# mazouziwissem/improving_yolov8_CBAM_SwinBlock

Hardware: AMD Instinct MI355X
Metric: images/sec fwd+bwd YOLOv8s-CBAM-Swin bs=32 640x640 (higher is better)
Workload: dtype bf16; 1 GPU; yolov8s.yaml (nc=1) forward + v8 loss + backward + clip + SGD-nesterov + EMA step, bs=32/GPU 640x640 (CBAM + 2x SwinBlock + SPPF5 + SPPF7); global_batch=32, imgsz=640, parallelism=dp1

## Files before the change

improving_yolov8_cbam_swinblock_amd/_lib.py:

```python
import ctypes
import os
import subprocess
import threading
from pathlib import Path

import torch

PKG_DIR = Path(__file__).resolve().parent
CSRC_DIR = PKG_DIR / "csrc"
LIB_PATH = Path(os.environ["YMI_LIB"]).resolve() if os.environ.get("YMI_LIB") else PKG_DIR / "libyolo_mi355.so"

YMI_F32, YMI_BF16 = 0, 1
ACT_NONE, ACT_SILU, ACT_GELU = 0, 1, 2

_c_i64 = ctypes.c_int64
_c_i32 = ctypes.c_int32
_c_f32 = ctypes.c_float
_vp = ctypes.c_void_p
_sz = ctypes.c_size_t


class YmiTensor(ctypes.Structure):
    _fields_ = [
        ("data", _vp),
# ... 51 lines not shown
    ),
    "ymi_first_conv_stat_blocks": (_c_i64, [_c_i64, _c_i64, _c_i64]),
    "ymi_first_conv_bn_act_fwd": (_c_i32, [_vp, _c_i64, _c_i64, _c_i64, _c_i64, _vp, _c_i64, _vp, _vp, _vp, _vp, _c_f32, _c_f32, _c_i32, _TP, _TP, _vp, _vp,
                                           _vp, _sz, _vp]),
    "ymi_first_conv_bwd_workspace": (_c_i64, [_c_i64, _c_i64, _c_i64, _c_i64]),
    "ymi_first_conv_bn_act_bwd": (_c_i32, [_TP, _vp, _c_i64, _c_i64, _vp, _vp, _vp, _vp, _c_i32, _TP, _vp, _vp, _vp, _vp, _sz, _vp, _vp]),
    "ymi_bn_act_bwd_pair": (_c_i32, [_TP, _TP, _vp, _vp, _vp, _vp, _c_i64, _vp, _vp, _c_i32, _TP, _vp, _vp, _vp, _sz, _vp]),
    "ymi_conv2d_bwd_data": (_c_i32, [_TP, _vp, _c_i64, _c_i64, _c_i64, _c_i64, _TP, _vp]),
    "ymi_conv2d_bwd_data_add": (_c_i32, [_TP, _vp, _c_i64, _c_i64, _c_i64, _c_i64, _TP, _TP, _TP, _vp]),
    "ymi_swin_mlp_fwd": (_c_i32, [_TP, _vp, _vp, _c_i64, _vp, _vp, _TP, _TP, _TP, _TP, _vp]),
    "ymi_swin_ln_mlp_supported": (_c_i32, [_c_i64, _c_i64, _c_i32]),
    "ymi_swin_ln_mlp_pack_elems": (_c_i64, [_c_i64, _c_i64]),
    "ymi_swin_ln_mlp_pre_elems": (_c_i64, [_c_i64, _c_i64]),
    "ymi_swin_ln_mlp_pack": (_c_i32, [_vp, _vp, _c_i64, _c_i64, _vp, _vp]),
    "ymi_swin_ln_mlp_fwd": (_c_i32, [_TP, _vp, _vp, _c_f32, _vp, _vp, _vp, _c_i64, _TP, _vp, _vp, _vp, _TP, _vp]),
    "ymi_swin_ln_mlp_bwd_data": (_c_i32, [_TP, _vp, _vp, _c_i64, _TP, _TP, _TP, _vp]),
    "ymi_swin_mlp_bwd_data": (_c_i32, [_TP, _vp, _TP, _TP, _vp, _TP, _TP, _TP, _vp]),
    "ymi_conv2d_bwd_weight": (_c_i32, [_TP, _TP, _c_i64, _c_i64, _c_i64, _c_i64, _c_i64, _vp, _vp, _vp, _sz, _vp]),
    "ymi_conv2d_bwd_weight_workspace": (_sz, [_c_i64, _c_i64, _c_i64, _c_i64, _c_i64]),
    "ymi_conv2d_bwd_weight_deferred": (_c_i32, [_TP, _TP, _c_i64, _c_i64, _c_i64, _c_i64, _c_i64, _vp, _vp, _vp, _sz, _vp, _vp]),
    "ymi_wgrad_hold": (_c_i32, [_c_i32]),
    "ymi_wgrad_reduce_batch": (_c_i32, [_vp, _c_i32, _vp, _vp]),
    "ymi_sppf_pool3_fwd": (_c_i32, [_TP, _c_i64, _TP, _TP, _TP, _vp]),
    "ymi_sppf_pool3_bwd_workspace": (_c_i64, [_c_i64, _c_i64, _c_i64, _c_i64, _c_i32]),
    "ymi_sppf_pool3_bwd": (_c_i32, [_TP, _TP, _TP, _c_i64, _TP, _TP, _TP, _TP, _TP, _vp, _c_i64, _vp]),
    "ymi_cbam_fwd": (_c_i32, [_TP, _vp, _vp, _c_i64, _vp, _c_i64, _TP, _vp, _vp, _vp, _vp, _vp, _vp, _vp]),
    "ymi_cbam_bwd": (_c_i32, [_TP, _TP, _vp, _vp, _c_i64, _vp, _c_i64, _vp, _vp, _vp, _vp, _vp, _vp, _TP, _vp, _vp, _vp, _vp, _sz, _vp]),
    "ymi_cbam_bwd_workspace": (_sz, [_c_i64, _c_i64, _c_i64, _c_i64, _c_i64]),
    "ymi_window_partition_index": (_c_i32, [_c_i64, _c_i64, _c_i64, _c_i64, _vp, _vp]),
    "ymi_window_partition": (_c_i32, [_TP, _c_i64, _TP, _vp]),
# ... 217 lines not shown
```

improving_yolov8_cbam_swinblock_amd/csrc/common.h:

```cpp
#pragma once
#include <hip/hip_runtime.h>
#include <stdint.h>
#include <stdio.h>

#include "../../include/ymi.h"

typedef __bf16 bf16_t;
typedef __attribute__((ext_vector_type(8))) __bf16 bf16x8;
typedef __attribute__((ext_vector_type(4))) __bf16 bf16x4;
typedef __attribute__((ext_vector_type(4))) float f32x4;
typedef __attribute__((ext_vector_type(2))) float f32x2;
typedef __attribute__((ext_vector_type(4))) uint32_t u32x4;
typedef __attribute__((ext_vector_type(2))) uint32_t u32x2;

typedef const __attribute__((address_space(1))) void* gptr_t;
typedef __attribute__((address_space(3))) void* lptr_t;

#define YMI_WAVE 64

void ymi_set_error(const char* fmt, ...);
#define YMI_CHECK_ARG(cond, ...)          \
    do {                                  \
        if (!(cond)) {                    \
            ymi_set_error(__VA_ARGS__);   \
// ... 325 lines not shown

template <int N> __device__ __forceinline__ void wait_vmcnt_barrier() {
    asm volatile("s_waitcnt vmcnt(%0)\n\ts_barrier" ::"n"(N) : "memory");
}

__device__ __forceinline__ float wave_sum(float v) {
#pragma unroll
    for (int o = 32; o > 0; o >>= 1) v += __shfl_xor(v, o, 64);
    return v;
}
__device__ __forceinline__ float wave_max(float v) {
#pragma unroll
    for (int o = 32; o > 0; o >>= 1) v = fmaxf(v, __shfl_xor(v, o, 64));
    return v;
}
```

improving_yolov8_cbam_swinblock_amd/csrc/swin.hip:

```cpp
#include <stdlib.h>

#include <type_traits>

#include "common.h"

struct SV {
    const void* p;
    int64_t ld;
};

__device__ __forceinline__ int64_t token_pixel(int64_t t64, int H, int W, int Hp, int Wp, int ws, bool* real) {
    const uint32_t t = (uint32_t)t64, L = (uint32_t)(ws * ws), uws = (uint32_t)ws;
    const uint32_t nww = (uint32_t)Wp / uws, nwh = (uint32_t)Hp / uws;
    const uint32_t win = t / L, tok = t - win * L;
    const uint32_t wrow = win / nww, ww = win - wrow * nww;
    const uint32_t b = wrow / nwh, wh = wrow - b * nwh;
    const uint32_t tr = tok / uws;
    const int h = (int)(wh * uws + tr), w = (int)(ww * uws + (tok - tr * uws));
    *real = (h < H) && (w < W);
    return ((int64_t)b * H + h) * W + w;
}

__global__ void window_index_kernel(int64_t T, int Hp, int Wp, int ws, int* __restrict__ out) {
    for (int64_t t = blockIdx.x * (int64_t)blockDim.x + threadIdx.x; t < T; t += (int64_t)gridDim.x * blockDim.x) {
        bool real;
        out[t] = (int)token_pixel(t, Hp, Wp, Hp, Wp, ws, &real);
    }
}

extern "C" int ymi_window_partition_index(int64_t n, int64_t hp, int64_t wp, int64_t ws, int32_t* index, void* stream) {
    YMI_CHECK_ARG(index && ws > 0 && hp % ws == 0 && wp % ws == 0 && n > 0, "window_partition_index: args");
    const int64_t T = n * hp * wp;
    YMI_CHECK_ARG(T < (1ll << 31), "window_partition_index: too many tokens");
    hipLaunchKernelGGL(window_index_kernel, dim3((unsigned)((T + 255) / 256 > 4096 ? 4096 : (T + 255) / 256)), dim3(256), 0, (hipStream_t)stream,
                       T, (int)hp, (int)wp, (int)ws, index);
    YMI_CHECK_LAUNCH("window_partition_index");
// ... 377 lines not shown

struct AttnLds {
    size_t stage;
    int nstage, nsq;
    size_t sq;
    bool tail;
    constexpr size_t region(int i) const { return (size_t)i * stage; }
    constexpr size_t square(int i) const { return (size_t)nstage * stage + (size_t)i * sq; }
    constexpr size_t floats() const { return square(nsq); }
    constexpr size_t bytes() const { return floats() + (tail ? 64 * sizeof(float) : 0); }
};
template <typename T> constexpr AttnLds attn_one_tile_lds(int hdp, bool bwd) {
    const int rows = 64 * attn_row_bytes<T>(hdp), cols = hdp * attn_row_bytes<T>(64);
    return AttnLds{(size_t)(rows > cols ? rows : cols), 2, bwd ? 3 : 1, (size_t)64 * attn_row_bytes<T>(64), bwd};
}
constexpr AttnLds attn_tr_lds(int hdp, bool bwd) {
    return AttnLds{(size_t)64 * attn_row_bytes<bf16_t>(hdp), bwd ? 4 : 3, bwd ? 2 : 1, (size_t)64 * attn_row_bytes<bf16_t>(64), false};
}
template <typename T> constexpr AttnLds attn_tiled_lds(int nsq) {
    constexpr int rows = 64 * attn_row_bytes<T>(ATT_HC), cols = ATT_HC * attn_row_bytes<T>(64);
    return AttnLds{(size_t)(rows > cols ? rows : cols), 2, nsq, (size_t)64 * attn_row_bytes<T>(64), true};
}
static_assert(attn_one_tile_lds<float>(attn_hdp(16 * ATT_MAXDT), true).bytes() <= ATT_LDS_MAX, "one-tile float32 backward image exceeds the LDS");
static_assert(attn_tr_lds(attn_hdp(16 * ATT_MAXDT), true).bytes() <= ATT_LDS_MAX, "tr backward image exceeds the LDS");
static_assert(attn_one_tile_lds<float>(192, true).bytes() == 156928 && attn_tr_lds(192, true).bytes() == 120832, "tests/attn_exact.py attn_lds restates these");
static_assert(attn_tiled_lds<float>(2).bytes() <= ATT_LDS_MAX, "tiled dK/dV image exceeds the LDS");

__device__ __forceinline__ void attn_softmax_row(f32x4 (&s)[4], int nkeys, float scale, float m_run, int l4, float& mx, float& sum) {
    mx = m_run;
#pragma unroll
    for (int t = 0; t < 4; ++t)
#pragma unroll
        for (int r = 0; r < 4; ++r) {
            const int j = 16 * t + 4 * l4 + r;
            s[t][r] = j < nkeys ? s[t][r] * scale : -__builtin_inff();
            mx = fmaxf(mx, s[t][r]);
        }
    mx = fmaxf(mx, __shfl_xor(mx, 16, 64));
    mx = fmaxf(mx, __shfl_xor(mx, 32, 64));
    sum = 0.f;
// ... 253 lines not shown
        }
    }
}

__global__ __launch_bounds__(256) void window_attn_fwd_tr_kernel(AttnArgs a) {
    typedef bf16_t T;
    extern __shared__ __attribute__((aligned(16))) char smem[];
    const int lane = threadIdx.x & 63, wv = threadIdx.x >> 6;
    const int l15 = lane & 15, l4 = lane >> 4;
    const int hdp = a.hdp, L = a.L;
    const int rstride = attn_row_bytes<T>(hdp), tstride = attn_row_bytes<T>(64);
    const AttnLds lds = attn_tr_lds(hdp, false);
    char* Qs = smem + lds.region(0);
    char* Ks = smem + lds.region(1);
    char* Vs = smem + lds.region(2);
    char* P = smem + lds.square(0);
    const int head = blockIdx.y;
    const int co = head * a.hd;
    const int64_t t0 = (int64_t)blockIdx.x * L;
    const T* qkv = reinterpret_cast<const T*>(a.qkv.p) + t0 * a.qkv.ld;
    T* out = reinterpret_cast<T*>(const_cast<void*>(a.out.p)) + t0 * a.out.ld;
    const int ndt = (a.hd + 15) / 16;
    const bool vec4 = (a.hd & 3) == 0 && (a.out.ld & 3) == 0 && (((uintptr_t)a.out.p) & 7) == 0;
    {
        const bf16_t* srcs[3] = {qkv + co, qkv + a.C + co, qkv + 2 * a.C + co};
        const int64_t lds_[3] = {a.qkv.ld, a.qkv.ld, a.qkv.ld};
        char* dsts[3] = {Qs, Ks, Vs};
        attn_stage_rows<3>(srcs, lds_, dsts, L, a.hd, hdp);
    }
    __syncthreads();
    f32x4 s[4];
#pragma unroll
    for (int t = 0; t < 4; ++t) {
        s[t] = f32x4{0.f, 0.f, 0.f, 0.f};
        AT<T>::mma(Ks, rstride, t * 16, Qs, rstride, wv * 16, hdp, lane, s[t]);
    }
    float mx, sum;
    attn_softmax_row(s, L, a.scale, -__builtin_inff(), l4, mx, sum);
    const float inv = 1.f / sum;
    const int m = 16 * wv + l15;
    if (l4 == 0 && m < L && a.lse) a.lse[(t0 + m) * a.heads + head] = mx + __logf(sum);
#pragma unroll
    for (int t = 0; t < 4; ++t) {
        float p[4];
#pragma unroll
        for (int r = 0; r < 4; ++r) p[r] = s[t][r] * inv;
        Pack<T, 4>::store(reinterpret_cast<T*>(P + (size_t)m * tstride) + 16 * t + 4 * l4, p);
    }
    __syncthreads();
#pragma unroll
    for (int dt = 0; dt < ATT_MAXDT; ++dt)
        if (dt < ndt) {
            f32x4 o = f32x4{0.f, 0.f, 0.f, 0.f};
#pragma unroll
            for (int k0 = 0; k0 < 64; k0 += 32) {
                const bf16x8 af = *reinterpret_cast<const bf16x8*>(P + (size_t)(16 * wv + l15) * tstride + (k0 + 8 * l4) * 2);
// ... 4 lines not shown
        }
}

__global__ __launch_bounds__(256) void window_attn_bwd_tr_kernel(AttnArgs a) {
    typedef bf16_t T;
    extern __shared__ __attribute__((aligned(16))) char smem[];
    const int lane = threadIdx.x & 63, wv = threadIdx.x >> 6;
    const int l15 = lane & 15, l4 = lane >> 4;
    const int hdp = a.hdp, L = a.L;
    const int rstride = attn_row_bytes<T>(hdp), tstride = attn_row_bytes<T>(64);
    const AttnLds lds = attn_tr_lds(hdp, true);
    char* Qs = smem + lds.region(0);
    char* Ks = smem + lds.region(1);
    char* Vs = smem + lds.region(2);
    char* Os = smem + lds.region(3);
    char* Ps = smem + lds.square(0);
    char* Ds = smem + lds.square(1);
    const int head = blockIdx.y;
    const int co = head * a.hd;
    const int64_t t0 = (int64_t)blockIdx.x * L;
    const T* qkv = reinterpret_cast<const T*>(a.qkv.p) + t0 * a.qkv.ld;
    const T* dO = reinterpret_cast<const T*>(a.dout.p) + t0 * a.dout.ld;
    T* dqkv = reinterpret_cast<T*>(const_cast<void*>(a.dqkv.p)) + t0 * a.dqkv.ld;
    const int ndt = (a.hd + 15) / 16;
    const bool vec4 = (a.hd & 3) == 0 && (a.C & 3) == 0 && (a.dqkv.ld & 3) == 0 && (((uintptr_t)a.dqkv.p) & 7) == 0;

    const int mrow = 16 * wv + l15;
    const float lse = mrow < L ? a.lse[(t0 + mrow) * a.heads + head] : 0.f;
    {
        const bf16_t* srcs[4] = {qkv + co, qkv + a.C + co, qkv + 2 * a.C + co, dO + co};
        const int64_t lds_[4] = {a.qkv.ld, a.qkv.ld, a.qkv.ld, a.dout.ld};
        char* dsts[4] = {Qs, Ks, Vs, Os};
// ... 7 lines not shown
        dp[t] = f32x4{0.f, 0.f, 0.f, 0.f};
        AT<T>::mma(Ks, rstride, t * 16, Qs, rstride, wv * 16, hdp, lane, s[t]);
        AT<T>::mma(Vs, rstride, t * 16, Os, rstride, wv * 16, hdp, lane, dp[t]);
    }
    float pr[4][4], delta = 0.f;
#pragma unroll
    for (int t = 0; t < 4; ++t)
#pragma unroll
        for (int r = 0; r < 4; ++r) {
            const bool ok = (16 * t + 4 * l4 + r < L) && (mrow < L);
            pr[t][r] = ok ? __expf(s[t][r] * a.scale - lse) : 0.f;
            delta += pr[t][r] * dp[t][r];
        }
    delta += __shfl_xor(delta, 16, 64);
    delta += __shfl_xor(delta, 32, 64);
#pragma unroll
    for (int t = 0; t < 4; ++t) {
        float ds[4];
#pragma unroll
        for (int r = 0; r < 4; ++r) ds[r] = pr[t][r] * (dp[t][r] - delta) * a.scale;
        Pack<T, 4>::store(reinterpret_cast<T*>(Ps + (size_t)mrow * tstride) + 16 * t + 4 * l4, pr[t]);
        Pack<T, 4>::store(reinterpret_cast<T*>(Ds + (size_t)mrow * tstride) + 16 * t + 4 * l4, ds);
    }
    __syncthreads();
#pragma unroll
    for (int dt = 0; dt < ATT_MAXDT; ++dt)
        if (dt < ndt) {
            f32x4 dv = f32x4{0.f, 0.f, 0.f, 0.f}, dk = dv, dq = dv;
#pragma unroll
            for (int k0 = 0; k0 < 64; k0 += 32) {
// ... 324 lines not shown
```

improving_yolov8_cbam_swinblock_amd/csrc/swin_mlp.hip:

```cpp
#include <type_traits>

#include "common.h"

typedef __attribute__((ext_vector_type(16))) float f32x16;

template <int I, int N, class F> __device__ __forceinline__ void static_for(F&& f) {
    if constexpr (I < N) {
        f(std::integral_constant<int, I>{});
        static_for<I + 1, N>(f);
    }
}

constexpr int MLP_PAD = 256;
constexpr int MLP_HC = 32;
constexpr int MLP_LDS_MAX = 160 * 1024;
template <int C> struct MlpCfg {
    static_assert(C == 128 || C == 256 || C == 384, "SwinBlock widths of the model files");
    static constexpr int NW = C > 256 ? 4 : 8;
    static constexpr int WPS = NW / 4;
    static constexpr bool HALVES = NW == 8;
    static constexpr int NT = NW * 64;
    static constexpr int BM = NW * 32;
    static constexpr int KS = C / 16;
    static constexpr int CT = C / 32;
// ... 37 lines not shown
    const float* gamma;
    const float* beta;
    float eps;
    const bf16_t* w1p;
    const bf16_t* w2q;
    const float* b1;
    const float* b2;
    bf16_t* u;
    int64_t ldu;
    float* mean;
    float* rstd;
    bf16_t* pre;
    bf16_t* out;
    int64_t ldo;
    int T, hidden;
};

__device__ __forceinline__ uint32_t pack_bf16x2(float a, float b) {
    typedef __attribute__((ext_vector_type(2))) __bf16 bf16x2;
    const bf16x2 v = {(bf16_t)a, (bf16_t)b};
    return __builtin_bit_cast(uint32_t, v);
}
__device__ __forceinline__ float bf16_lo(uint32_t v) { return __builtin_bit_cast(float, v << 16); }
__device__ __forceinline__ float bf16_hi(uint32_t v) { return __builtin_bit_cast(float, v & 0xffff0000u); }

__device__ __forceinline__ float gelu_fast(float x, float* half_erfc = nullptr, float* e_out = nullptr) {
    const float ax = fabsf(x);
    const float t = __builtin_amdgcn_rcpf(fmaf(0.3275911f * 0.70710678118654752440f, ax, 1.0f));
    const float s = ax * 0.84932180028801904272f;
    const float e = __builtin_amdgcn_exp2f(-(s * s));
// ... 74 lines not shown
            acc[i >> 1] = __builtin_amdgcn_mfma_f32_32x32x16_bf16(f[i & 3], hv[i & 1], acc[i >> 1], 0, 0, 0);
        }
        __builtin_amdgcn_sched_barrier(0);
        if constexpr (i + 4 < 2 * CT) MLP_RD(f[i & 3], ad, (i + 4) * 1024);
    });
}

template <int C> __device__ __forceinline__ int mlp_swz(int idx, int r) { return C == 256 ? idx ^ r : idx ^ (r & 15); }

template <int CT> __device__ __forceinline__ void mlp_settle_acc() {
    if constexpr (CT > 8) asm volatile("s_nop 7\n\ts_nop 7\n\ts_nop 1" ::: "memory");
}

template <int C, bool SKIP>
__device__ __forceinline__ void mlp_store_tile(f32x16 (&acc)[C / 32], const float* bias, const bf16_t* skip, int64_t ldskip, bf16_t* dst, int64_t ldd, int row0,
                                               int T, char* img, int lane) {
    constexpr int ROWB = 2 * C, CPR = C / 8;
    const int px = lane & 31, h = lane >> 5;
    const int row = row0 + px;
    const bool rok = row < T;
    const int rowc = rok ? row : T - 1;
#pragma unroll
    for (int ct = 0; ct < C / 32; ++ct) {
#pragma unroll
        for (int q = 0; q < 4; ++q) {
            const int ch = 32 * ct + 8 * q + 4 * h;
            float v[4];
            const f32x4 bb = bias ? *reinterpret_cast<const f32x4*>(bias + ch) : f32x4{0.f, 0.f, 0.f, 0.f};
#pragma unroll
            for (int r = 0; r < 4; ++r) v[r] = acc[ct][4 * q + r] + bb[r];
            if (SKIP) {
                const u32x2 s = *reinterpret_cast<const u32x2*>(skip + (int64_t)rowc * ldskip + ch);
                v[0] += bf16_lo(s[0]); v[1] += bf16_hi(s[0]); v[2] += bf16_lo(s[1]); v[3] += bf16_hi(s[1]);
            }
            u32x2 o;
            o[0] = pack_bf16x2(v[0], v[1]);
            o[1] = pack_bf16x2(v[2], v[3]);
            *reinterpret_cast<u32x2*>(img + px * ROWB + 16 * mlp_swz<C>(4 * ct + q, px) + 8 * h) = o;
        }
    }
#pragma unroll
    for (int i = 0; i < C / 16; ++i) {
        const int r = CPR == 32 ? 2 * i + h : (64 * i + lane) / CPR, cl = CPR == 32 ? px : (64 * i + lane) % CPR;
        const u32x4 val = *reinterpret_cast<const u32x4*>(img + r * ROWB + 16 * mlp_swz<C>(cl, r));
        if (row0 + r < T) *reinterpret_cast<u32x4*>(dst + (int64_t)(row0 + r) * ldd + cl * 8) = val;
    }
}

template <int KS> __device__ __forceinline__ void mlp_forget(bf16x8 (&v)[KS]) {
    if constexpr (KS > 16) {
#pragma unroll
        for (int s = 0; s < KS; ++s) asm volatile("" : "+v"(v[s]));
    }
}

__device__ __forceinline__ void mlp_barrier() { asm volatile("s_barrier" ::: "memory"); }

template <int C> __global__ __launch_bounds__(MlpCfg<C>::NT, MlpCfg<C>::WPS) void swin_mlp_fwd_kernel(MlpFwdArgs a) {
    using K = MlpCfg<C>;
    constexpr int KS = K::KS, CT = K::CT, NW = K::NW, MLP_STAGE = K::STAGE;
// ... 144 lines not shown
            hv[0] = __builtin_bit_cast(bf16x8, t0);
            hv[1] = __builtin_bit_cast(bf16x8, t1);
            mlp_barrier();
            if (jc + 2 < nch) mlp_issue<C>(a.w1p, a.w2q, jc + 2, smem + ((jc + 2) % 3) * MLP_STAGE, tid, wave);
            __builtin_amdgcn_s_setprio(1);
            mlp_cols_product<CT>(lds0 + (jc % 3) * MLP_STAGE + K::IMG, hv, acc);
            if (jc + 1 < nch) {
                bias_tile(jc + 1, d1);
                mlp_rows_product<KS>(lds0 + ((jc + 1) % 3) * MLP_STAGE, uf, d1);
            }
            __builtin_amdgcn_s_setprio(0);
            mlp_barrier();
        }
    }
    mlp_settle_acc<CT>();
    mlp_store_tile<C, true>(acc, a.b2, a.x, a.ldx, a.out, a.ldo, row0, a.T, smem + wave * (32 * K::ROWB), lane);
}

struct MlpBwdArgs {
    const bf16_t* dout;
    int64_t lddo;
    const bf16_t* w2t;
    const bf16_t* w1tq;
    const bf16_t* pre;
    bf16_t* post;
    int64_t ldpost;
    bf16_t* dpre;
    int64_t lddpre;
    bf16_t* du;
    int64_t lddu;
    int T, hidden;
// ... 70 lines not shown
            hf[i] = pack_bf16x2(dp[0], dp[1]);
        }
#pragma unroll
        for (int g = 0; g < 2; ++g) {
            *reinterpret_cast<u32x4*>(post_base + (size_t)(jc * 64 + 16 * g) + row_off) = u32x4{of[4 * g], of[4 * g + 1], of[4 * g + 2], of[4 * g + 3]};
            *reinterpret_cast<u32x4*>(dpre_base + (size_t)(jc * 64 + 16 * g) + row_off) = u32x4{hf[4 * g], hf[4 * g + 1], hf[4 * g + 2], hf[4 * g + 3]};
        }
        u32x4 t0 = {hf[0], hf[1], hf[2], hf[3]}, t1 = {hf[4], hf[5], hf[6], hf[7]};
        hv[0] = __builtin_bit_cast(bf16x8, t0);
        hv[1] = __builtin_bit_cast(bf16x8, t1);
        if (half == 0) asm volatile("s_waitcnt vmcnt(6)" ::: "memory");
        mlp_barrier();
    }
    if (K::HALVES && half == 0) mlp_barrier();
    mlp_settle_acc<CT>();
    mlp_store_tile<C, false>(acc, nullptr, nullptr, 0, a.du, a.lddu, row0, a.T, smem + wave * (32 * K::ROWB), lane);
}

template <int C> static void mlp_launch_fwd(const MlpFwdArgs& a, hipStream_t stream) {
    using K = MlpCfg<C>;
    const size_t lds = K::LDS_TILE + (size_t)a.hidden * sizeof(float);
    (void)hipFuncSetAttribute(reinterpret_cast<const void*>(swin_mlp_fwd_kernel<C>), hipFuncAttributeMaxDynamicSharedMemorySize, (int)lds);
    hipLaunchKernelGGL(swin_mlp_fwd_kernel<C>, dim3((unsigned)((a.T + K::BM - 1) / K::BM)), dim3(K::NT), lds, stream, a);
}
template <int C> static void mlp_launch_bwd(const MlpBwdArgs& a, hipStream_t stream) {
    using K = MlpCfg<C>;
    const size_t lds = K::LDS_TILE;
    (void)hipFuncSetAttribute(reinterpret_cast<const void*>(swin_mlp_bwd_kernel<C>), hipFuncAttributeMaxDynamicSharedMemorySize, (int)lds);
    hipLaunchKernelGGL(swin_mlp_bwd_kernel<C>, dim3((unsigned)((a.T + K::BM - 1) / K::BM)), dim3(K::NT), lds, stream, a);
}
#define MLP_WIDTHS "128, 256 or 384"
// ... 5 lines not shown
extern "C" int64_t ymi_swin_ln_mlp_pack_elems(int64_t c, int64_t hidden) { return 4 * c * hidden; }
extern "C" int64_t ymi_swin_ln_mlp_pre_elems(int64_t tokens, int64_t hidden) { return (tokens + MLP_PAD - 1) / MLP_PAD * MLP_PAD * hidden; }

extern "C" int ymi_swin_ln_mlp_pack(const float* w1, const float* w2, int64_t c, int64_t hidden, void* packed, void* stream) {
    YMI_CHECK_ARG(w1 && w2 && packed && ymi_swin_ln_mlp_supported(c, hidden, YMI_BF16),
                  "swin_ln_mlp_pack: C = " MLP_WIDTHS ", hidden a multiple of %d up to %d / %d / %d", MLP_HC, MlpCfg<128>::HIDDEN_MAX, MlpCfg<256>::HIDDEN_MAX,
                  MlpCfg<384>::HIDDEN_MAX);
    YMI_CHECK_ARG(((uintptr_t)packed & 15) == 0, "swin_ln_mlp_pack: 16-byte alignment");
    const int64_t n = c * hidden;
    hipLaunchKernelGGL(swin_mlp_pack_kernel, dim3((unsigned)((n + 255) / 256 < 1024 ? (n + 255) / 256 : 1024)), dim3(256), 0, (hipStream_t)stream, w1, w2, (int)c, (int)hidden,
                       (bf16_t*)packed);
    YMI_CHECK_LAUNCH("swin_ln_mlp_pack");
    return YMI_OK;
}

extern "C" int ymi_swin_ln_mlp_fwd(const ymi_tensor* x, const float* gamma, const float* beta, float eps, const void* packed, const float* b1, const float* b2,
                                   int64_t hidden, const ymi_tensor* u, float* mean, float* rstd, void* pre, const ymi_tensor* out, void* stream) {
    YMI_CHECK_ARG(ymi_tensor_ok(x) && ymi_tensor_ok(out) && gamma && beta && packed && b1 && b2, "swin_ln_mlp_fwd: args");
    YMI_CHECK_ARG(ymi_swin_ln_mlp_supported(x->c, hidden, x->dtype) && out->dtype == x->dtype && out->c == x->c && ymi_pixels(out) == ymi_pixels(x),
                  "swin_ln_mlp_fwd: bfloat16 tokens of " MLP_WIDTHS " channels, hidden a multiple of %d up to %d / %d / %d", MLP_HC, MlpCfg<128>::HIDDEN_MAX,
                  MlpCfg<256>::HIDDEN_MAX, MlpCfg<384>::HIDDEN_MAX);
    const bool train = u != nullptr;
    if (train) YMI_CHECK_ARG(ymi_tensor_ok(u) && u->dtype == x->dtype && u->c == x->c && ymi_pixels(u) == ymi_pixels(x) && mean && rstd && pre, "swin_ln_mlp_fwd: saved tensors");
    YMI_CHECK_ARG(x->ld % 8 == 0 && out->ld % 8 == 0 && (!train || u->ld % 8 == 0) && ((((uintptr_t)x->data) | ((uintptr_t)out->data) | ((uintptr_t)packed) |
                  ((uintptr_t)gamma) | ((uintptr_t)beta) | ((uintptr_t)b1) | ((uintptr_t)b2) | (train ? ((uintptr_t)u->data | (uintptr_t)pre) : 0)) & 15) == 0,
                  "swin_ln_mlp_fwd: 16-byte alignment");
    const int64_t T = ymi_pixels(x);
    YMI_CHECK_ARG(T < (1ll << 31) && T * x->ld < (1ll << 31), "swin_ln_mlp_fwd: too large");
    const int64_t n = x->c * hidden;
    MlpFwdArgs a{};
    a.x = (const bf16_t*)x->data; a.ldx = x->ld;
    a.gamma = gamma; a.beta = beta; a.eps = eps;
    a.w1p = (const bf16_t*)packed; a.w2q = a.w1p + n;
    a.b1 = b1; a.b2 = b2;
    a.u = train ? (bf16_t*)u->data : nullptr; a.ldu = train ? u->ld : 0;
    a.mean = mean; a.rstd = rstd; a.pre = (bf16_t*)pre;
    a.out = (bf16_t*)out->data; a.ldo = out->ld;
    a.T = (int)T; a.hidden = (int)hidden;
    if (x->c == 128) mlp_launch_fwd<128>(a, (hipStream_t)stream);
    else if (x->c == 256) mlp_launch_fwd<256>(a, (hipStream_t)stream);
    else mlp_launch_fwd<384>(a, (hipStream_t)stream);
    YMI_CHECK_LAUNCH("swin_ln_mlp_fwd");
    return YMI_OK;
}

extern "C" int ymi_swin_ln_mlp_bwd_data(const ymi_tensor* dout, const void* packed, const void* pre, int64_t hidden, const ymi_tensor* post, const ymi_tensor* dpre,
                                        const ymi_tensor* du, void* stream) {
    YMI_CHECK_ARG(ymi_tensor_ok(dout) && ymi_tensor_ok(post) && ymi_tensor_ok(dpre) && ymi_tensor_ok(du) && packed && pre, "swin_ln_mlp_bwd_data: args");
    const int64_t T = ymi_pixels(dout);
    YMI_CHECK_ARG(ymi_swin_ln_mlp_supported(dout->c, hidden, dout->dtype) && post->dtype == dout->dtype && dpre->dtype == dout->dtype && du->dtype == dout->dtype &&
                      post->c == hidden && dpre->c == hidden && du->c == dout->c && ymi_pixels(post) == T && ymi_pixels(dpre) == T && ymi_pixels(du) == T,
                  "swin_ln_mlp_bwd_data: shapes (bfloat16 tokens of " MLP_WIDTHS " channels)");
    YMI_CHECK_ARG(dout->ld % 8 == 0 && du->ld % 8 == 0 && post->ld % 4 == 0 && dpre->ld % 4 == 0 &&
                      ((((uintptr_t)dout->data) | ((uintptr_t)du->data) | ((uintptr_t)packed) | ((uintptr_t)pre)) & 15) == 0 &&
                      ((((uintptr_t)post->data) | ((uintptr_t)dpre->data)) & 15) == 0,
                  "swin_ln_mlp_bwd_data: alignment");
    YMI_CHECK_ARG(T < (1ll << 31) && (T + MLP_PAD) * post->ld < (1ll << 31), "swin_ln_mlp_bwd_data: too large");
    YMI_CHECK_ARG(post->ld == hidden && dpre->ld == hidden, "swin_ln_mlp_bwd_data: post / dpre are dense [T][hidden] views of buffers of ymi_swin_ln_mlp_pre_elems elements");
// ... 16 lines not shown
```

improving_yolov8_cbam_swinblock_amd/nn/modules/swin_block.py:

```python
import torch.nn as nn

from ... import ops


def window_partition(x, window_size):
    b, h, w, c = x.shape
    xi = ops.to_internal(x.permute(0, 3, 1, 2))
    return ops.window_partition(xi, window_size).view(-1, window_size * window_size, c)


def window_reverse(windows, window_size, H, W):
    c = windows.shape[-1]
    b = int(windows.shape[0] / (H * W / window_size / window_size))
    t = windows.reshape(-1, c)
    return ops.window_reverse(t, b, H, W, window_size).permute(0, 2, 3, 1)


class SwinBlock(nn.Module):

    def __init__(self, dim, num_heads=2, window_size=7):
        super().__init__()
        self.dim = dim
        self.window_size = window_size
        self.norm1 = nn.LayerNorm(dim)
# ... 4 lines not shown
    def forward(self, x, out=None):
        x = ops.to_internal(x)
        n, c, h, w = x.shape
        ws = self.window_size
        if c != self.dim:
            raise RuntimeError(f"Given normalized_shape=[{self.dim}], expected input with {self.dim} channels, got {c}")
        a = self.attn
        join = self.training
        t1 = ops.layernorm(x, self.norm1, ws)
        if join:
            ops.mark_join(t1, 2)
        qkv = ops.linear(t1, a.in_proj_weight, a.in_proj_bias)
        o = ops.window_attention(qkv, ws * ws, a.num_heads)
        t2 = ops.linear(o, a.out_proj.weight, a.out_proj.bias, residual=t1)
        if ops.swin_ln_mlp_ok(t2, self.mlp[0]) and self.mlp[0].bias is not None and self.mlp[2].bias is not None:
            t3 = ops.swin_ln_mlp(t2, self.norm2, self.mlp[0], self.mlp[2])
        else:
            if join:
                ops.mark_join(t2, 2)
            u = ops.layernorm(t2, self.norm2, 0)
            t3 = ops.swin_mlp(u, self.mlp[0], self.mlp[2], residual=t2)
        return ops.window_reverse(t3, n, h, w, ws, out)
```

improving_yolov8_cbam_swinblock_amd/ops/base.py:

```python
import ctypes
import os

import torch

from .. import _lib
from .._lib import ACT_GELU, ACT_NONE, ACT_SILU, ConvProblem, DgradProblem, as_ymi, check, chunk_elems, empty_nhwc, is_nhwc, ptr, stream_ptr, workspace, ymi_dtype

_byref = ctypes.byref


def L():
    return _lib.lib()


HOOKS = {
    "fused_swin_mlp": True,
    "detect_pair": True,
    "detect_multi": True,
    "first_conv": True,
    "stat_atomics": True,
    "wgrad_rider": True,
}


def compute_dtype(x):
    if torch.is_autocast_enabled("cuda") if hasattr(torch, "is_autocast_enabled") else False:
        dt = torch.get_autocast_dtype("cuda")
        if dt != torch.bfloat16:
            raise RuntimeError(f"libyolo_mi355 supports bfloat16 autocast only (got {dt}); fp16 has no kernels here")
        return dt
    return x.dtype if x.dtype in (torch.float32, torch.bfloat16) else torch.float32
# ... 255 lines not shown
```

improving_yolov8_cbam_swinblock_amd/ops/blocks.py:

```python
import ctypes
import os

import torch

from .. import _lib
from .._lib import ACT_GELU, ACT_NONE, ACT_SILU, ConvProblem, DgradProblem, as_ymi, check, chunk_elems, empty_nhwc, is_nhwc, ptr, stream_ptr, workspace, ymi_dtype
from .base import (
    HOOKS, L, _accumulate, _byref, _dense_ok, _join_plain, _note_use, _prep_adds, grad_nhwc, join_of, round_up,
)
from .weights import (
    _wgrad_maybe_async, pack_conv_dgrad, pack_conv_fwd,
)
from .conv import (
    padded_grad_like,
)

LN_BWD_MAX_BLOCKS = 2048


def _layernorm_bwd(x, ws, dy, gamma, stats, add, dx):
    c = x.shape[1]
    dgb = torch.empty((2, c), dtype=torch.float32, device=x.device)
    wsb = workspace(LN_BWD_MAX_BLOCKS * 2 * c * 4 + 256, x.device, "ln")
    check(
# ... 78 lines not shown
    return _SwinMlp.apply(u, fc1.weight, fc1.bias, fc2.weight, fc2.bias, residual, join_of(u), join_of(residual) if residual is not None else None)


FUSED_SWIN_MLP_WIDTHS = (256,)


def swin_ln_mlp_ok(x, fc1):
    return (HOOKS["fused_swin_mlp"] and x.dim() == 2 and x.is_cuda and x.dtype == torch.bfloat16 and x.stride(1) == 1 and x.stride(0) % 8 == 0
            and x.shape[1] in FUSED_SWIN_MLP_WIDTHS and bool(L().ymi_swin_ln_mlp_supported(x.shape[1], fc1.weight.shape[0], ymi_dtype(x.dtype))))



class _SwinLnMlp(torch.autograd.Function):

    @staticmethod
    def forward(ctx, x, gamma, beta, eps, w1, b1, w2, b2):
        t, c = x.shape
        hidden = w1.shape[0]
        dev = x.device
        lib = L()
        _note_use(w1, w2)
        packed = torch.empty(lib.ymi_swin_ln_mlp_pack_elems(c, hidden), dtype=torch.bfloat16, device=dev)
        check(lib.ymi_swin_ln_mlp_pack(ptr(w1.detach()), ptr(w2.detach()), c, hidden, ptr(packed), stream_ptr()), "swin_ln_mlp_pack")
        train = any(ctx.needs_input_grad)
        out = torch.empty((t, c), dtype=x.dtype, device=dev)
        u = torch.empty((t, c), dtype=x.dtype, device=dev) if train else None
        stats = torch.empty((2, t), dtype=torch.float32, device=dev) if train else None
        pre = torch.empty(lib.ymi_swin_ln_mlp_pre_elems(t, hidden), dtype=x.dtype, device=dev) if train else None
        check(
            lib.ymi_swin_ln_mlp_fwd(_byref(as_ymi(x)), ptr(gamma), ptr(beta), eps, ptr(packed), ptr(b1), ptr(b2), hidden, _byref(as_ymi(u)) if train else None,
                                    ptr(stats[0]) if train else None, ptr(stats[1]) if train else None, ptr(pre), _byref(as_ymi(out)), stream_ptr()),
            "swin_ln_mlp_fwd",
        )
        if train:
            ctx.save_for_backward(x, gamma, w1, w2, u, stats, pre, packed)
            ctx.biases = (b1, b2)
        return out

    @staticmethod
    def backward(ctx, dout):
        x, gamma, w1, w2, u, stats, pre, packed = ctx.saved_tensors
        b1, b2 = ctx.biases
        dtype = x.dtype
        dev = x.device
        t, c = x.shape
        hidden = w1.shape[0]
        dout = grad_nhwc(dout, dtype)
        cap = L().ymi_swin_ln_mlp_pre_elems(t, hidden)
        post = torch.empty(cap, dtype=dtype, device=dev).view(-1, hidden)[:t]
        dpre = torch.empty(cap, dtype=dtype, device=dev).view(-1, hidden)[:t]
        du = torch.empty((t, c), dtype=dtype, device=dev)
        check(L().ymi_swin_ln_mlp_bwd_data(_byref(as_ymi(dout)), ptr(packed), ptr(pre), hidden, _byref(as_ymi(post)), _byref(as_ymi(dpre)), _byref(as_ymi(du)),
                                           stream_ptr()), "swin_ln_mlp_bwd_data")
        dw1, db1, dw2, db2 = _mlp_wgrads(u, dpre, post, dout, w1, b1, w2, b2, ctx.needs_input_grad[4:8])
        dx = torch.empty_like(x)
        dgamma, dbeta = _layernorm_bwd(x, 0, du, gamma, stats, dout, dx)
        return dx, dgamma, dbeta, None, dw1, db1, dw2, db2


def swin_ln_mlp(x, ln, fc1, fc2):
    return _SwinLnMlp.apply(x, ln.weight, ln.bias, float(ln.eps), fc1.weight, fc1.bias, fc2.weight, fc2.bias)


class _Act(torch.autograd.Function):

    @staticmethod
    def forward(ctx, pre, act):
        out = torch.empty_like(pre)
        check(L().ymi_scale_shift_act(_byref(as_ymi(pre)), None, None, act, None, _byref(as_ymi(out)), stream_ptr()), "scale_shift_act")
        ctx.save_for_backward(pre)
        ctx.act = act
        return out

    @staticmethod
    def backward(ctx, dy):
        (pre,) = ctx.saved_tensors
# ... 438 lines not shown
```

include/ymi.h:

```cpp
#ifndef YMI_H
#define YMI_H

#include <stddef.h>
#include <stdint.h>

#ifdef __cplusplus
extern "C" {
#endif

#define YMI_VERSION 1

enum { YMI_F32 = 0, YMI_BF16 = 1 };
enum { YMI_ACT_NONE = 0, YMI_ACT_SILU = 1, YMI_ACT_GELU = 2 };
enum { YMI_OK = 0, YMI_EINVAL = -1, YMI_EALIGN = -2, YMI_ELAUNCH = -3, YMI_EWORKSPACE = -4 };

typedef struct ymi_tensor {
    void* data;
    int64_t n, h, w, c;
    int64_t ld;
    int32_t dtype;
    int32_t _pad;
} ymi_tensor;

int ymi_version(void);
// ... 247 lines not shown
                   const float* const* host_grads, const float* hyper, const void* state, int32_t rule, void* stream);
int ymi_opt_grad_accumulate(const ymi_opt_entry* table, const int32_t* chunk_map, int32_t first_tensor, int32_t n_tensors, int64_t n_chunks,
                            const float* const* host_grads, void* stream);

int ymi_swin_mlp_fwd(const ymi_tensor* u, const void* w1_packed, const float* b1, int64_t hidden, const void* w2_packed, const float* b2,
                     const ymi_tensor* residual, const ymi_tensor* pre, const ymi_tensor* post, const ymi_tensor* out, void* stream);
int ymi_swin_mlp_bwd_data(const ymi_tensor* dout, const void* w2_dgrad_packed, const ymi_tensor* pre, const ymi_tensor* dpre,
                          const void* w1_dgrad_packed, const ymi_tensor* add1, const ymi_tensor* add2, const ymi_tensor* du, void* stream);

int ymi_swin_ln_mlp_supported(int64_t c, int64_t hidden, int32_t dtype);
int64_t ymi_swin_ln_mlp_pack_elems(int64_t c, int64_t hidden);
int64_t ymi_swin_ln_mlp_pre_elems(int64_t tokens, int64_t hidden);
int ymi_swin_ln_mlp_pack(const float* w1, const float* w2, int64_t c, int64_t hidden, void* packed, void* stream);
int ymi_swin_ln_mlp_fwd(const ymi_tensor* x, const float* gamma, const float* beta, float eps, const void* packed, const float* b1, const float* b2,
                        int64_t hidden, const ymi_tensor* u, float* mean, float* rstd, void* pre, const ymi_tensor* out, void* stream);
int ymi_swin_ln_mlp_bwd_data(const ymi_tensor* dout, const void* packed, const void* pre, int64_t hidden, const ymi_tensor* post, const ymi_tensor* dpre,
                             const ymi_tensor* du, void* stream);

#ifdef __cplusplus
}
#endif
#endif
```

Before: 2741 images/sec.

## Scatter Swin MLP output directly to image layout and alias attention P in LDS

The fused LN+MLP forward kernel can now write its output straight into the NHWC image using window-to-pixel indexing. This removes the separate window-reverse pass and drops padded tokens, and the backward re-partitions the incoming gradient to match. Separately, the tr attention kernels reuse the K or V LDS region for the P tile when it fits. That shrinks the LDS footprint so more blocks can share a CU, at the cost of an extra barrier.

Measured after the change: 2760 images/sec (median of 6 runs). No clear change (+0.7%).

```diff
diff --git a/improving_yolov8_cbam_swinblock_amd/_lib.py b/improving_yolov8_cbam_swinblock_amd/_lib.py
--- a/improving_yolov8_cbam_swinblock_amd/_lib.py
+++ b/improving_yolov8_cbam_swinblock_amd/_lib.py
@@ -89,6 +89,7 @@
     "ymi_swin_ln_mlp_pre_elems": (_c_i64, [_c_i64, _c_i64]),
     "ymi_swin_ln_mlp_pack": (_c_i32, [_vp, _vp, _c_i64, _c_i64, _vp, _vp]),
     "ymi_swin_ln_mlp_fwd": (_c_i32, [_TP, _vp, _vp, _c_f32, _vp, _vp, _vp, _c_i64, _TP, _vp, _vp, _vp, _TP, _vp]),
+    "ymi_swin_ln_mlp_fwd_windows": (_c_i32, [_TP, _vp, _vp, _c_f32, _vp, _vp, _vp, _c_i64, _TP, _vp, _vp, _vp, _c_i64, _TP, _vp]),
     "ymi_swin_ln_mlp_bwd_data": (_c_i32, [_TP, _vp, _vp, _c_i64, _TP, _TP, _TP, _vp]),
     "ymi_swin_mlp_bwd_data": (_c_i32, [_TP, _vp, _TP, _TP, _vp, _TP, _TP, _TP, _vp]),
     "ymi_conv2d_bwd_weight": (_c_i32, [_TP, _TP, _c_i64, _c_i64, _c_i64, _c_i64, _c_i64, _vp, _vp, _vp, _sz, _vp]),
diff --git a/improving_yolov8_cbam_swinblock_amd/csrc/common.h b/improving_yolov8_cbam_swinblock_amd/csrc/common.h
--- a/improving_yolov8_cbam_swinblock_amd/csrc/common.h
+++ b/improving_yolov8_cbam_swinblock_amd/csrc/common.h
@@ -363,3 +363,15 @@
     for (int o = 32; o > 0; o >>= 1) v = fmaxf(v, __shfl_xor(v, o, 64));
     return v;
 }
+
+__device__ __forceinline__ int64_t token_pixel(int64_t t64, int H, int W, int Hp, int Wp, int ws, bool* real) {
+    const uint32_t t = (uint32_t)t64, L = (uint32_t)(ws * ws), uws = (uint32_t)ws;
+    const uint32_t nww = (uint32_t)Wp / uws, nwh = (uint32_t)Hp / uws;
+    const uint32_t win = t / L, tok = t - win * L;
+    const uint32_t wrow = win / nww, ww = win - wrow * nww;
+    const uint32_t b = wrow / nwh, wh = wrow - b * nwh;
+    const uint32_t tr = tok / uws;
+    const int h = (int)(wh * uws + tr), w = (int)(ww * uws + (tok - tr * uws));
+    *real = (h < H) && (w < W);
+    return ((int64_t)b * H + h) * W + w;
+}
diff --git a/improving_yolov8_cbam_swinblock_amd/csrc/swin.hip b/improving_yolov8_cbam_swinblock_amd/csrc/swin.hip
--- a/improving_yolov8_cbam_swinblock_amd/csrc/swin.hip
+++ b/improving_yolov8_cbam_swinblock_amd/csrc/swin.hip
@@ -9,17 +9,6 @@
     int64_t ld;
 };
 
-__device__ __forceinline__ int64_t token_pixel(int64_t t64, int H, int W, int Hp, int Wp, int ws, bool* real) {
-    const uint32_t t = (uint32_t)t64, L = (uint32_t)(ws * ws), uws = (uint32_t)ws;
-    const uint32_t nww = (uint32_t)Wp / uws, nwh = (uint32_t)Hp / uws;
-    const uint32_t win = t / L, tok = t - win * L;
-    const uint32_t wrow = win / nww, ww = win - wrow * nww;
-    const uint32_t b = wrow / nwh, wh = wrow - b * nwh;
-    const uint32_t tr = tok / uws;
-    const int h = (int)(wh * uws + tr), w = (int)(ww * uws + (tok - tr * uws));
-    *real = (h < H) && (w < W);
-    return ((int64_t)b * H + h) * W + w;
-}
 
 __global__ void window_index_kernel(int64_t T, int Hp, int Wp, int ws, int* __restrict__ out) {
     for (int64_t t = blockIdx.x * (int64_t)blockDim.x + threadIdx.x; t < T; t += (int64_t)gridDim.x * blockDim.x) {
@@ -427,8 +416,10 @@
     const int rows = 64 * attn_row_bytes<T>(hdp), cols = hdp * attn_row_bytes<T>(64);
     return AttnLds{(size_t)(rows > cols ? rows : cols), 2, bwd ? 3 : 1, (size_t)64 * attn_row_bytes<T>(64), bwd};
 }
+constexpr bool attn_tr_p_aliased(int hdp) { return attn_row_bytes<bf16_t>(hdp) >= attn_row_bytes<bf16_t>(64); }
 constexpr AttnLds attn_tr_lds(int hdp, bool bwd) {
-    return AttnLds{(size_t)64 * attn_row_bytes<bf16_t>(hdp), bwd ? 4 : 3, bwd ? 2 : 1, (size_t)64 * attn_row_bytes<bf16_t>(64), false};
+    return AttnLds{(size_t)64 * attn_row_bytes<bf16_t>(hdp), bwd ? 4 : 3, (bwd ? 2 : 1) - (attn_tr_p_aliased(hdp) ? 1 : 0),
+                   (size_t)64 * attn_row_bytes<bf16_t>(64), false};
 }
 template <typename T> constexpr AttnLds attn_tiled_lds(int nsq) {
     constexpr int rows = 64 * attn_row_bytes<T>(ATT_HC), cols = ATT_HC * attn_row_bytes<T>(64);
@@ -436,7 +427,11 @@
 }
 static_assert(attn_one_tile_lds<float>(attn_hdp(16 * ATT_MAXDT), true).bytes() <= ATT_LDS_MAX, "one-tile float32 backward image exceeds the LDS");
 static_assert(attn_tr_lds(attn_hdp(16 * ATT_MAXDT), true).bytes() <= ATT_LDS_MAX, "tr backward image exceeds the LDS");
-static_assert(attn_one_tile_lds<float>(192, true).bytes() == 156928 && attn_tr_lds(192, true).bytes() == 120832, "tests/attn_exact.py attn_lds restates these");
+static_assert(attn_one_tile_lds<float>(192, true).bytes() == 156928, "tests/attn_exact.py attn_lds restates this");
+static_assert(attn_tr_lds(192, true).bytes() == 120832 - 9216 && attn_tr_lds(32, true).bytes() == 38912 && attn_tr_lds(32, false).bytes() == 24576,
+              "tests/attn_exact.py attn_lds is an upper bound of the tr images: P's square less where it is aliased, the same at head_dim <= 32");
+static_assert(2 * attn_tr_lds(128, true).bytes() <= ATT_LDS_MAX && attn_tr_lds(128, true).bytes() == 78848, "two tr backward images at head_dim 128 must share a CU");
+static_assert(3 * attn_tr_lds(128, false).bytes() <= ATT_LDS_MAX && attn_tr_lds(128, false).bytes() == 52224, "three tr forward images at head_dim 128 must share a CU");
 static_assert(attn_tiled_lds<float>(2).bytes() <= ATT_LDS_MAX, "tiled dK/dV image exceeds the LDS");
 
 __device__ __forceinline__ void attn_softmax_row(f32x4 (&s)[4], int nkeys, float scale, float m_run, int l4, float& mx, float& sum) {
@@ -720,7 +715,7 @@
     char* Qs = smem + lds.region(0);
     char* Ks = smem + lds.region(1);
     char* Vs = smem + lds.region(2);
-    char* P = smem + lds.square(0);
+    char* P = attn_tr_p_aliased(hdp) ? Ks : smem + lds.square(0);
     const int head = blockIdx.y;
     const int co = head * a.hd;
     const int64_t t0 = (int64_t)blockIdx.x * L;
@@ -746,6 +741,7 @@
     const float inv = 1.f / sum;
     const int m = 16 * wv + l15;
     if (l4 == 0 && m < L && a.lse) a.lse[(t0 + m) * a.heads + head] = mx + __logf(sum);
+    __syncthreads();
 #pragma unroll
     for (int t = 0; t < 4; ++t) {
         float p[4];
@@ -780,8 +776,8 @@
     char* Ks = smem + lds.region(1);
     char* Vs = smem + lds.region(2);
     char* Os = smem + lds.region(3);
-    char* Ps = smem + lds.square(0);
-    char* Ds = smem + lds.square(1);
+    char* Ds = smem + lds.square(0);
+    char* Ps = attn_tr_p_aliased(hdp) ? Vs : smem + lds.square(1);
     const int head = blockIdx.y;
     const int co = head * a.hd;
     const int64_t t0 = (int64_t)blockIdx.x * L;
@@ -819,6 +815,7 @@
         }
     delta += __shfl_xor(delta, 16, 64);
     delta += __shfl_xor(delta, 32, 64);
+    __syncthreads();
 #pragma unroll
     for (int t = 0; t < 4; ++t) {
         float ds[4];
diff --git a/improving_yolov8_cbam_swinblock_amd/csrc/swin_mlp.hip b/improving_yolov8_cbam_swinblock_amd/csrc/swin_mlp.hip
--- a/improving_yolov8_cbam_swinblock_amd/csrc/swin_mlp.hip
+++ b/improving_yolov8_cbam_swinblock_amd/csrc/swin_mlp.hip
@@ -75,6 +75,7 @@
     bf16_t* out;
     int64_t ldo;
     int T, hidden;
+    int H, W, Hp, Wp, ws;
 };
 
 __device__ __forceinline__ uint32_t pack_bf16x2(float a, float b) {
@@ -179,7 +180,7 @@
 
 template <int C, bool SKIP>
 __device__ __forceinline__ void mlp_store_tile(f32x16 (&acc)[C / 32], const float* bias, const bf16_t* skip, int64_t ldskip, bf16_t* dst, int64_t ldd, int row0,
-                                               int T, char* img, int lane) {
+                                               int T, int drow, char* img, int lane) {
     constexpr int ROWB = 2 * C, CPR = C / 8;
     const int px = lane & 31, h = lane >> 5;
     const int row = row0 + px;
@@ -208,7 +209,8 @@
     for (int i = 0; i < C / 16; ++i) {
         const int r = CPR == 32 ? 2 * i + h : (64 * i + lane) / CPR, cl = CPR == 32 ? px : (64 * i + lane) % CPR;
         const u32x4 val = *reinterpret_cast<const u32x4*>(img + r * ROWB + 16 * mlp_swz<C>(cl, r));
-        if (row0 + r < T) *reinterpret_cast<u32x4*>(dst + (int64_t)(row0 + r) * ldd + cl * 8) = val;
+        const int dr = __shfl(drow, r, 64);
+        if (dr >= 0) *reinterpret_cast<u32x4*>(dst + (int64_t)dr * ldd + cl * 8) = val;
     }
 }
 
@@ -383,7 +385,13 @@
         }
     }
     mlp_settle_acc<CT>();
-    mlp_store_tile<C, true>(acc, a.b2, a.x, a.ldx, a.out, a.ldo, row0, a.T, smem + wave * (32 * K::ROWB), lane);
+    int drow = rok ? row : -1;
+    if (a.ws > 0 && rok) {
+        bool real;
+        const int pixel = (int)token_pixel(row, a.H, a.W, a.Hp, a.Wp, a.ws, &real);
+        drow = real ? pixel : -1;
+    }
+    mlp_store_tile<C, true>(acc, a.b2, a.x, a.ldx, a.out, a.ldo, row0, a.T, drow, smem + wave * (32 * K::ROWB), lane);
 }
 
 struct MlpBwdArgs {
@@ -484,7 +492,7 @@
     }
     if (K::HALVES && half == 0) mlp_barrier();
     mlp_settle_acc<CT>();
-    mlp_store_tile<C, false>(acc, nullptr, nullptr, 0, a.du, a.lddu, row0, a.T, smem + wave * (32 * K::ROWB), lane);
+    mlp_store_tile<C, false>(acc, nullptr, nullptr, 0, a.du, a.lddu, row0, a.T, row < a.T ? row : -1, smem + wave * (32 * K::ROWB), lane);
 }
 
 template <int C> static void mlp_launch_fwd(const MlpFwdArgs& a, hipStream_t stream) {
@@ -520,19 +528,20 @@
     return YMI_OK;
 }
 
-extern "C" int ymi_swin_ln_mlp_fwd(const ymi_tensor* x, const float* gamma, const float* beta, float eps, const void* packed, const float* b1, const float* b2,
-                                   int64_t hidden, const ymi_tensor* u, float* mean, float* rstd, void* pre, const ymi_tensor* out, void* stream) {
-    YMI_CHECK_ARG(ymi_tensor_ok(x) && ymi_tensor_ok(out) && gamma && beta && packed && b1 && b2, "swin_ln_mlp_fwd: args");
-    YMI_CHECK_ARG(ymi_swin_ln_mlp_supported(x->c, hidden, x->dtype) && out->dtype == x->dtype && out->c == x->c && ymi_pixels(out) == ymi_pixels(x),
-                  "swin_ln_mlp_fwd: bfloat16 tokens of " MLP_WIDTHS " channels, hidden a multiple of %d up to %d / %d / %d", MLP_HC, MlpCfg<128>::HIDDEN_MAX,
-                  MlpCfg<256>::HIDDEN_MAX, MlpCfg<384>::HIDDEN_MAX);
+static int mlp_fwd(const char* what, const ymi_tensor* x, const float* gamma, const float* beta, float eps, const void* packed, const float* b1, const float* b2,
+                   int64_t hidden, const ymi_tensor* u, float* mean, float* rstd, void* pre, int64_t ws, const ymi_tensor* out, void* stream) {
+    YMI_CHECK_ARG(ymi_tensor_ok(x) && ymi_tensor_ok(out) && gamma && beta && packed && b1 && b2 && ws >= 0, "%s: args", what);
+    const int64_t T = ymi_pixels(x);
+    const int64_t Hp = ws ? (out->h + ws - 1) / ws * ws : 0, Wp = ws ? (out->w + ws - 1) / ws * ws : 0;
+    YMI_CHECK_ARG(ymi_swin_ln_mlp_supported(x->c, hidden, x->dtype) && out->dtype == x->dtype && out->c == x->c && (ws ? out->n * Hp * Wp : ymi_pixels(out)) == T,
+                  "%s: bfloat16 tokens of " MLP_WIDTHS " channels, hidden a multiple of %d up to %d / %d / %d%s", what, MLP_HC, MlpCfg<128>::HIDDEN_MAX,
+                  MlpCfg<256>::HIDDEN_MAX, MlpCfg<384>::HIDDEN_MAX, ws ? "; one token per pixel of the image padded to whole windows" : "");
     const bool train = u != nullptr;
-    if (train) YMI_CHECK_ARG(ymi_tensor_ok(u) && u->dtype == x->dtype && u->c == x->c && ymi_pixels(u) == ymi_pixels(x) && mean && rstd && pre, "swin_ln_mlp_fwd: saved tensors");
+    if (train) YMI_CHECK_ARG(ymi_tensor_ok(u) && u->dtype == x->dtype && u->c == x->c && ymi_pixels(u) == ymi_pixels(x) && mean && rstd && pre, "%s: saved tensors", what);
     YMI_CHECK_ARG(x->ld % 8 == 0 && out->ld % 8 == 0 && (!train || u->ld % 8 == 0) && ((((uintptr_t)x->data) | ((uintptr_t)out->data) | ((uintptr_t)packed) |
                   ((uintptr_t)gamma) | ((uintptr_t)beta) | ((uintptr_t)b1) | ((uintptr_t)b2) | (train ? ((uintptr_t)u->data | (uintptr_t)pre) : 0)) & 15) == 0,
-                  "swin_ln_mlp_fwd: 16-byte alignment");
-    const int64_t T = ymi_pixels(x);
-    YMI_CHECK_ARG(T < (1ll << 31) && T * x->ld < (1ll << 31), "swin_ln_mlp_fwd: too large");
+                  "%s: 16-byte alignment", what);
+    YMI_CHECK_ARG(T < (1ll << 31) && T * x->ld < (1ll << 31), "%s: too large", what);
     const int64_t n = x->c * hidden;
     MlpFwdArgs a{};
     a.x = (const bf16_t*)x->data; a.ldx = x->ld;
@@ -543,11 +552,21 @@
     a.mean = mean; a.rstd = rstd; a.pre = (bf16_t*)pre;
     a.out = (bf16_t*)out->data; a.ldo = out->ld;
     a.T = (int)T; a.hidden = (int)hidden;
+    a.H = (int)out->h; a.W = (int)out->w; a.Hp = (int)Hp; a.Wp = (int)Wp; a.ws = (int)ws;
     if (x->c == 128) mlp_launch_fwd<128>(a, (hipStream_t)stream);
     else if (x->c == 256) mlp_launch_fwd<256>(a, (hipStream_t)stream);
     else mlp_launch_fwd<384>(a, (hipStream_t)stream);
-    YMI_CHECK_LAUNCH("swin_ln_mlp_fwd");
+    YMI_CHECK_LAUNCH(what);
     return YMI_OK;
+}
+extern "C" int ymi_swin_ln_mlp_fwd(const ymi_tensor* x, const float* gamma, const float* beta, float eps, const void* packed, const float* b1, const float* b2,
+                                   int64_t hidden, const ymi_tensor* u, float* mean, float* rstd, void* pre, const ymi_tensor* out, void* stream) {
+    return mlp_fwd("swin_ln_mlp_fwd", x, gamma, beta, eps, packed, b1, b2, hidden, u, mean, rstd, pre, 0, out, stream);
+}
+extern "C" int ymi_swin_ln_mlp_fwd_windows(const ymi_tensor* x, const float* gamma, const float* beta, float eps, const void* packed, const float* b1, const float* b2,
+                                           int64_t hidden, const ymi_tensor* u, float* mean, float* rstd, void* pre, int64_t ws, const ymi_tensor* image, void* stream) {
+    YMI_CHECK_ARG(ws > 0, "swin_ln_mlp_fwd_windows: window size");
+    return mlp_fwd("swin_ln_mlp_fwd_windows", x, gamma, beta, eps, packed, b1, b2, hidden, u, mean, rstd, pre, ws, image, stream);
 }
 
 extern "C" int ymi_swin_ln_mlp_bwd_data(const ymi_tensor* dout, const void* packed, const void* pre, int64_t hidden, const ymi_tensor* post, const ymi_tensor* dpre,
diff --git a/improving_yolov8_cbam_swinblock_amd/nn/modules/swin_block.py b/improving_yolov8_cbam_swinblock_amd/nn/modules/swin_block.py
--- a/improving_yolov8_cbam_swinblock_amd/nn/modules/swin_block.py
+++ b/improving_yolov8_cbam_swinblock_amd/nn/modules/swin_block.py
@@ -42,6 +42,8 @@
         o = ops.window_attention(qkv, ws * ws, a.num_heads)
         t2 = ops.linear(o, a.out_proj.weight, a.out_proj.bias, residual=t1)
         if ops.swin_ln_mlp_ok(t2, self.mlp[0]) and self.mlp[0].bias is not None and self.mlp[2].bias is not None:
+            if ops.HOOKS["swin_mlp_scatter"]:
+                return ops.swin_ln_mlp(t2, self.norm2, self.mlp[0], self.mlp[2], windows=(n, h, w, ws, out))
             t3 = ops.swin_ln_mlp(t2, self.norm2, self.mlp[0], self.mlp[2])
         else:
             if join:
diff --git a/improving_yolov8_cbam_swinblock_amd/ops/base.py b/improving_yolov8_cbam_swinblock_amd/ops/base.py
--- a/improving_yolov8_cbam_swinblock_amd/ops/base.py
+++ b/improving_yolov8_cbam_swinblock_amd/ops/base.py
@@ -15,6 +15,7 @@
 
 HOOKS = {
     "fused_swin_mlp": True,
+    "swin_mlp_scatter": True,
     "detect_pair": True,
     "detect_multi": True,
     "first_conv": True,
diff --git a/improving_yolov8_cbam_swinblock_amd/ops/blocks.py b/improving_yolov8_cbam_swinblock_amd/ops/blocks.py
--- a/improving_yolov8_cbam_swinblock_amd/ops/blocks.py
+++ b/improving_yolov8_cbam_swinblock_amd/ops/blocks.py
@@ -116,7 +116,7 @@
 class _SwinLnMlp(torch.autograd.Function):
 
     @staticmethod
-    def forward(ctx, x, gamma, beta, eps, w1, b1, w2, b2):
+    def forward(ctx, x, gamma, beta, eps, w1, b1, w2, b2, windows=None):
         t, c = x.shape
         hidden = w1.shape[0]
         dev = x.device
@@ -125,15 +125,22 @@
         packed = torch.empty(lib.ymi_swin_ln_mlp_pack_elems(c, hidden), dtype=torch.bfloat16, device=dev)
         check(lib.ymi_swin_ln_mlp_pack(ptr(w1.detach()), ptr(w2.detach()), c, hidden, ptr(packed), stream_ptr()), "swin_ln_mlp_pack")
         train = any(ctx.needs_input_grad)
-        out = torch.empty((t, c), dtype=x.dtype, device=dev)
+        if windows is None:
+            out = torch.empty((t, c), dtype=x.dtype, device=dev)
+        else:
+            n, h, w, ws, slot = windows
+            out = slot.view(n, c, h, w, x.dtype) if slot is not None else empty_nhwc(n, c, h, w, x.dtype, dev)
         u = torch.empty((t, c), dtype=x.dtype, device=dev) if train else None
         stats = torch.empty((2, t), dtype=torch.float32, device=dev) if train else None
         pre = torch.empty(lib.ymi_swin_ln_mlp_pre_elems(t, hidden), dtype=x.dtype, device=dev) if train else None
-        check(
-            lib.ymi_swin_ln_mlp_fwd(_byref(as_ymi(x)), ptr(gamma), ptr(beta), eps, ptr(packed), ptr(b1), ptr(b2), hidden, _byref(as_ymi(u)) if train else None,
-                                    ptr(stats[0]) if train else None, ptr(stats[1]) if train else None, ptr(pre), _byref(as_ymi(out)), stream_ptr()),
-            "swin_ln_mlp_fwd",
-        )
+        saved = (_byref(as_ymi(u)) if train else None, ptr(stats[0]) if train else None, ptr(stats[1]) if train else None, ptr(pre))
+        if windows is None:
+            check(lib.ymi_swin_ln_mlp_fwd(_byref(as_ymi(x)), ptr(gamma), ptr(beta), eps, ptr(packed), ptr(b1), ptr(b2), hidden, *saved, _byref(as_ymi(out)),
+                                          stream_ptr()), "swin_ln_mlp_fwd")
+        else:
+            check(lib.ymi_swin_ln_mlp_fwd_windows(_byref(as_ymi(x)), ptr(gamma), ptr(beta), eps, ptr(packed), ptr(b1), ptr(b2), hidden, *saved, windows[3],
+                                                  _byref(as_ymi(out)), stream_ptr()), "swin_ln_mlp_fwd_windows")
+        ctx.ws = 0 if windows is None else windows[3]
         if train:
             ctx.save_for_backward(x, gamma, w1, w2, u, stats, pre, packed)
             ctx.biases = (b1, b2)
@@ -148,6 +155,9 @@
         t, c = x.shape
         hidden = w1.shape[0]
         dout = grad_nhwc(dout, dtype)
+        if ctx.ws:
+            g, dout = dout, torch.empty((t, c), dtype=dtype, device=dev)
+            check(L().ymi_window_partition(_byref(as_ymi(g)), ctx.ws, _byref(as_ymi(dout)), stream_ptr()), "window_partition")
         cap = L().ymi_swin_ln_mlp_pre_elems(t, hidden)
         post = torch.empty(cap, dtype=dtype, device=dev).view(-1, hidden)[:t]
         dpre = torch.empty(cap, dtype=dtype, device=dev).view(-1, hidden)[:t]
@@ -157,11 +167,14 @@
         dw1, db1, dw2, db2 = _mlp_wgrads(u, dpre, post, dout, w1, b1, w2, b2, ctx.needs_input_grad[4:8])
         dx = torch.empty_like(x)
         dgamma, dbeta = _layernorm_bwd(x, 0, du, gamma, stats, dout, dx)
-        return dx, dgamma, dbeta, None, dw1, db1, dw2, db2
-
-
-def swin_ln_mlp(x, ln, fc1, fc2):
-    return _SwinLnMlp.apply(x, ln.weight, ln.bias, float(ln.eps), fc1.weight, fc1.bias, fc2.weight, fc2.bias)
+        return dx, dgamma, dbeta, None, dw1, db1, dw2, db2, None
+
+
+def swin_ln_mlp(x, ln, fc1, fc2, windows=None):
+    if windows is not None:
+        n, h, w, ws, slot = windows
+        windows = (int(n), int(h), int(w), int(ws), slot)
+    return _SwinLnMlp.apply(x, ln.weight, ln.bias, float(ln.eps), fc1.weight, fc1.bias, fc2.weight, fc2.bias, windows)
 
 
 class _Act(torch.autograd.Function):
diff --git a/include/ymi.h b/include/ymi.h
--- a/include/ymi.h
+++ b/include/ymi.h
@@ -285,6 +285,8 @@
 int ymi_swin_ln_mlp_pack(const float* w1, const float* w2, int64_t c, int64_t hidden, void* packed, void* stream);
 int ymi_swin_ln_mlp_fwd(const ymi_tensor* x, const float* gamma, const float* beta, float eps, const void* packed, const float* b1, const float* b2,
                         int64_t hidden, const ymi_tensor* u, float* mean, float* rstd, void* pre, const ymi_tensor* out, void* stream);
+int ymi_swin_ln_mlp_fwd_windows(const ymi_tensor* x, const float* gamma, const float* beta, float eps, const void* packed, const float* b1, const float* b2,
+                                int64_t hidden, const ymi_tensor* u, float* mean, float* rstd, void* pre, int64_t ws, const ymi_tensor* image, void* stream);
 int ymi_swin_ln_mlp_bwd_data(const ymi_tensor* dout, const void* packed, const void* pre, int64_t hidden, const ymi_tensor* post, const ymi_tensor* dpre,
                              const ymi_tensor* du, void* stream);
 
```
